# DavidPeicho/loupiote

Measured on AMD Instinct MI355X. Metric: Mrays/s (+ ms/frame) at 1920×1080, 4 spp, Sponza; 1/2/4/8 GPU, higher is better.
Workload: dtype f32

## Files before the change

loupiote_amd/csrc/device.hip:

```cpp
#include <hip/hip_runtime.h>

#include <dlfcn.h>

#include <algorithm>
#include <cmath>
#include <map>
#include <memory>
#include <cstdlib>
#include <functional>
#include <mutex>
#include <new>
#include <numeric>

#include "common.h"
#include "env_dist.h"
#include "emit_dist.h"
#include "material_tables.h"
#include "kernels.h"
#include "probe_kernels.h"
#include "build_kernels.h"
#include "launch_plan.h"
#include <hipcub/hipcub.hpp>
#include <rccl/rccl.h>

// ... 1887 lines not shown
                with_flags([&](auto D, auto L) { hipLaunchKernelGGL((k_raygen<decltype(D)::value, decltype(L)::value>), dim3(pl.stream_blocks), dim3(kBlock), 0, s, p, nz, w->q[0], w->Lsum, w->ctr); }, f.dense, f.lens);
                stage_end(r, s, slot);
                if (ph.wait_trav) HIP_TRY(hipStreamWaitEvent(s, ph.wait_trav, 0));
                if (pl.packet) {
                    stage_begin(r, ST_PRIMARY, s, slot);
                    with_flags([&](auto S) { hipLaunchKernelGGL(k_trace_packet<decltype(S)::value>, dim3(pl.packet_blocks), dim3(kTraceBlock), pl.packet_lds, s, sc, w->q[0], w->hits, w->ctr, 0, pl.quad_slots); }, f.stats);
                    stage_end(r, s, slot);
                } else if (pl.coop_all || !pl.path) trace(0, -1);
                if (pl.path) {
                    stage_begin(r, ST_PATH, s, slot);
                    const size_t plds = pl.stack_lds + kPathLdsExtra;
                    const float4 *h0 = pl.packet ? w->hits : (const float4 *)nullptr;
                    with_flags([&](auto G, auto S, auto P) {
                        auto launch = [&](auto... e) { hipLaunchKernelGGL((k_path<decltype(G)::value, decltype(S)::value, sizeof...(e) != 0, decltype(P)::value, decltype(e)...>), dim3(pl.path_blocks), dim3(kTraceBlock), plds, s, sc, probe, nz, p, w->q[0], h0, w->Lsum, w->ctr, seed0, gb, tune.path_refill, e...); };
                        if (f.env) launch(ev); else launch();
                    }, f.denoise, f.stats, f.punct);
                    stage_end(r, s, slot);
                }
            } else if (!pl.path) {
                const uint32_t b = t - 1u;
                const uint32_t seed = seed0 + t;
                const Queue qin = w->q[b & 1u], qout = w->q[(b + 1u) & 1u];
                stage_begin(r, ST_SHADE, s, slot);
                with_flags([&](auto G, auto P, auto Tr, auto Em, auto Es, auto Nm) {
                    auto launch = [&](auto... e) { hipLaunchKernelGGL((k_shade<decltype(G)::value, sizeof...(e) != 0, decltype(P)::value, decltype(Tr)::value, decltype(Em)::value, decltype(Em)::value && decltype(Es)::value, decltype(Nm)::value, decltype(e)...>), dim3(pl.shade_blocks), dim3(kBlock), 0, s, sc, probe, nz, p, qin, w->hits, qout, w->sq, w->Lsum, w->ctr, (int)b, seed, gb, sort_queues, e...); };
                    if (f.env) launch(ev); else launch();
                }, f.denoise && b == 0u, f.punct, f.trans, f.emis, esamp, f.nmap);
                stage_end(r, s, slot);
                if (ph.wait_trav) HIP_TRY(hipStreamWaitEvent(s, ph.wait_trav, 0));
                trace(b + 1u < nb ? (int)(b + 1u) : -1, (int)b);
            }
            if (ph.rec_trav) HIP_TRY(hipEventRecord(ph.rec_trav, s));
            if (t == nb && split) HIP_TRY(hipEventRecord(w->done, s));
            HIP_TRY(hipGetLastError());
            return LPT_OK;
        };
        for (uint32_t t = 0; !defer && t < tk.stages; ++t) {
            const int st = tk.run(t, PhaseHooks{});
            if (st != LPT_OK) return st;
        }
    }
    tk.p = p; tk.lane = lane; tk.split = split; tk.denoise = denoise; tk.cur = gb.cur;
    return LPT_OK;
}

static int wavefront_finish(lpt_renderer *r, const Ticket &tk, const ReadPlan *read, uint32_t row0, uint32_t row1) {
    hipStream_t sm = r->stream;
    const FrameParams &p = tk.p;
    Wavefront &wf = r->wf[tk.lane];
    const bool split = tk.split;
// ... 806 lines not shown
```

loupiote_amd/csrc/kernels.h:

```cpp
#pragma once
#include "device_math.h"

namespace lptd {

constexpr int kMaxBounces = 64;
constexpr int kBlock = 256;
constexpr int kTraceBlock = 64;

struct DNode8 {
    uint4 n0;
    uint4 n2;
    uint4 n3;
    uint4 n4;
};
using lpt::kNodeTris;

__device__ __forceinline__ uint32_t node_imask(const uint4 &n0) { return (n0.z >> 8) & 0xFFu; }
__device__ __forceinline__ uint32_t node_leaves(const uint4 &n0) { return n0.z >> 16; }
__device__ __forceinline__ uint32_t leaf_count(uint32_t V, uint32_t slot) { return 1u + ((V >> (8u + slot)) & 1u); }
struct NodeGrid { float px, py, pz, sx, sy, sz; };
template <typename Scene>
__device__ __forceinline__ NodeGrid node_grid(const Scene &sc, const uint4 &n0) {
    NodeGrid g;
    g.px = fmaf((float)(n0.x & 0xFFFFu), sc.grid_step[0], sc.grid_lo[0]);
// ... 143 lines not shown
        const uint32_t j = k - period * p.map.w;
#pragma unroll
        for (uint32_t q = 1; q < kMaxWeight; ++q) v = j == q ? p.map.vlist[q] : v;
    }
    const uint32_t tile = period * p.map.V + v;
    if (tile >= p.n_tiles) return false;
    const uint32_t ty = tile / p.tiles_x, tx = tile - ty * p.tiles_x;
    uint32_t wx, wy;
    within_to_xy(p, within, wx, wy);
    x = tx * p.tile_w + wx;
    y = ty * p.tile_h + wy;
    return x < p.width && y < p.height;
}

__device__ __forceinline__ uint32_t wave_compact(bool valid, uint32_t *counter) {
    const unsigned long long mask = __ballot(valid);
    const uint32_t lane = threadIdx.x & 63u;
    uint32_t base = 0;
    if (lane == 0 && mask) base = atomicAdd(counter, (uint32_t)__popcll(mask));
    base = __shfl(base, 0);
    return base + (uint32_t)__popcll(mask & ((1ull << lane) - 1ull));
}

__device__ __forceinline__ uint32_t block_compact(bool valid, uint32_t *counter, uint32_t *lds) {
    const unsigned long long mask = __ballot(valid);
    const uint32_t lane = threadIdx.x & 63u, wave = threadIdx.x >> 6;
    const uint32_t n = (uint32_t)__popcll(mask);
    if (lane == 0) lds[wave] = n;
    __syncthreads();
    if (threadIdx.x == 0) {
        const uint32_t n0 = lds[0], n1 = lds[1], n2 = lds[2], n3 = lds[3];
        const uint32_t total = n0 + n1 + n2 + n3;
        const uint32_t base = total ? atomicAdd(counter, total) : 0u;
        lds[4] = base; lds[5] = base + n0; lds[6] = base + n0 + n1; lds[7] = base + n0 + n1 + n2;
    }
    __syncthreads();
    const uint32_t idx = lds[4 + wave] + (uint32_t)__popcll(mask & ((1ull << lane) - 1ull));
    __syncthreads();
    return idx;
}

__device__ __forceinline__ uint32_t block_compact_binned(bool valid, uint32_t key, uint32_t *counter, uint32_t *lds) {
    const uint32_t lane = threadIdx.x & 63u, wave = threadIdx.x >> 6;
    unsigned long long mine = 0ull;
    uint32_t cnt_k = 0;
#pragma unroll
    for (uint32_t k = 0; k < 8u; ++k) {
        const unsigned long long m = __ballot(valid && key == k);
        if (key == k) mine = m;
        if (lane == k) cnt_k = (uint32_t)__popcll(m);
    }
    if (lane < 8u) lds[lane * 4u + wave] = cnt_k;
    __syncthreads();
    if (threadIdx.x < 32u) {
        const uint32_t c = lds[threadIdx.x];
        uint32_t incl = c;
#pragma unroll
        for (int off = 1; off < 32; off <<= 1) {
            const uint32_t v = __shfl_up(incl, off);
            if ((int)lane >= off) incl += v;
        }
        lds[32u + threadIdx.x] = incl - c;
        if (threadIdx.x == 31u) lds[64u] = incl ? atomicAdd(counter, incl) : 0u;
    }
    __syncthreads();
    const uint32_t idx = lds[64u] + lds[32u + key * 4u + wave] + (uint32_t)__popcll(mine & ((1ull << lane) - 1ull));
    __syncthreads();
    return idx;
}
__device__ __forceinline__ uint32_t dir_octant(float x, float y, float z) { return (x < 0.0f ? 1u : 0u) | (y < 0.0f ? 2u : 0u) | (z < 0.0f ? 4u : 0u); }

__device__ __forceinline__ void noise_shift(const DNoise &nz, uint32_t x, uint32_t y, uint32_t seed_counter, float &r0, float &r1) {
    if (!nz.enabled) return;
    const uint8_t *t = nz.rgba + 4u * ((size_t)(y % nz.h) * nz.w + (x % nz.w));
    float g = (float)(seed_counter & 1023u) * 0.61803398875f;
    float a = r0 + ((float)t[0] + 0.5f) * 0.00390625f + g;
    float b = r1 + ((float)t[1] + 0.5f) * 0.00390625f + g;
    a = a - floorf(a);
    b = b - floorf(b);
    if (a >= 1.0f) a = 0.0f;
    if (b >= 1.0f) b = 0.0f;
    r0 = a;
    r1 = b;
}

template <bool DENSE, bool LENS = false>
// ... 1197 lines not shown
    float4 no4, nd4, nT4;
    float4 so4, sd4, sc4;
};

struct PunctPick { float p_p, p_pick; };
template <bool ENV, bool ESAMP = false>
__device__ __forceinline__ PunctPick punct_pick(const DScene &sc) {
    PunctPick pk;
    pk.p_p = (float)sc.n_punctual / (float)(sc.n_punctual + sc.n_lights);
    pk.p_pick = (((ENV ? 0.5f : 1.0f) * (ESAMP ? 0.5f : 1.0f)) * pk.p_p) / (float)sc.n_punctual;
    return pk;
}
template <bool ENV, bool PUNCT, bool ESAMP = false>
__device__ __forceinline__ float rect_inv_nl(const DScene &sc, const PunctPick &pk) {
    if (PUNCT) return sc.n_lights ? (((ENV ? 0.5f : 1.0f) * (ESAMP ? 0.5f : 1.0f)) * (1.0f - pk.p_p)) / (float)sc.n_lights : 0.0f;
    return sc.n_lights ? ((ENV ? 0.5f : 1.0f) * (ESAMP ? 0.5f : 1.0f)) / (float)sc.n_lights : 0.0f;
}
template <bool ENV, bool ESAMP>
__device__ __forceinline__ float light_rl(const float r0, const float p_env, const float p_m) {
    float rl = ENV ? (r0 - p_env) / (1.0f - p_env) : r0;
    if (ESAMP) rl = (rl - p_m) / (1.0f - p_m);
    return rl;
}
template <bool GBUF, bool ENV, bool PUNCT, bool TRANS = false, bool EMIS = false, bool ESAMP = false, bool NMAP = false, typename LoadO, typename AddL>
__device__ __forceinline__ void shade_hit(const DScene &sc, const DProbe &probe, const DEnv &ev, const DNoise &nz, const FrameParams &p, const float *s_lut,
                                          const uint32_t bounce, const bool last_bounce, const uint32_t seed_base, const float inv_nl, const PunctPick &pk, const GBufArgs &gb,
                                          const float4 d4, const float4 T4, const float4 h4, LoadO load_o, AddL add_l, ShadeOut &out) {
    out.want_next = false; out.want_shadow = false; out.is_surface = false;
    const uint32_t pxy = __float_as_uint(T4.w);
    const f3 d = mk3(d4.x, d4.y, d4.z);
    const f3 T = mk3(T4.x, T4.y, T4.z);
    const uint32_t prim = __float_as_uint(h4.w);
    f3 g_n = neg(d), g_alb = mk3(1.0f, 1.0f, 1.0f);
    f3 g_P = mk3(0.f, 0.f, 0.f);
    if (GBUF && bounce == 0) {
        const float4 o4 = load_o();
        g_P = mk3(fmaf(d.x, h4.x, o4.x), fmaf(d.y, h4.x, o4.y), fmaf(d.z, h4.x, o4.z));
    }
    if (prim == 0xFFFFFFFFu) {
        f3 e = env_lookup(probe, d);
        if (ENV) {
            const float pdf_prev = load_o().w;
            if (pdf_prev >= 0.0f) {
                const float pe = ((PUNCT || ESAMP || sc.n_lights) ? 0.5f : 1.0f) * env_pdf(ev, d);
                const float pb2 = pdf_prev * pdf_prev;
                const float w = pb2 / (pb2 + pe * pe);
                e = mk3(e.x * w, e.y * w, e.z * w);
            }
        }
        add_l(T.x * e.x, T.y * e.y, T.z * e.z);
    } else if (prim & LPT_LIGHT_BIT) {
        const float4 *Lt = reinterpret_cast<const float4 *>(sc.lights + (prim & ~LPT_LIGHT_BIT));
        const float4 n4 = Lt[0], t4 = Lt[1], b4 = Lt[2], lo4 = Lt[3];
        const float Le = lo4.w;
        g_n = mk3(n4.x, n4.y, n4.z);
        float w = 1.0f;
        const float pdf_prev = load_o().w;
        if (pdf_prev >= 0.0f) {
            float cl = -dot(mk3(n4.x, n4.y, n4.z), d);
            float area = 4.0f * (t4.w * b4.w);
            float pl = ((h4.x * h4.x) / (cl * area)) * inv_nl;
            float pb2 = pdf_prev * pdf_prev;
            w = pb2 / (pb2 + pl * pl);
        }
        float k = Le * w;
        add_l(T.x * k, T.y * k, T.z * k);
    } else {
        const float hu = h4.y, hv = h4.z;
        const float4 *tv = sc.tri_verts + kTriRec * (size_t)prim;
        const float4 P0 = tv[0], N0 = tv[1], P1 = tv[2], N1 = tv[3], P2 = tv[4], N2 = tv[5];
        const float4 mc = tv[6], mp = tv[7];
        uint32_t em = 0u;
        if (EMIS) em = sc.emis_tri[prim];
        uint32_t nm = 0u;
        if (NMAP) nm = sc.nmap_tri[prim];
        float bw = (1.0f - hu) - hv;
        const f3 p0 = mk3(P0.x, P0.y, P0.z), p1 = mk3(P1.x, P1.y, P1.z), p2 = mk3(P2.x, P2.y, P2.z);
        f3 P = mk3((p0.x * bw + p1.x * hu) + p2.x * hv, (p0.y * bw + p1.y * hu) + p2.y * hv, (p0.z * bw + p1.z * hu) + p2.z * hv);
        f3 Ng = cross(p1 - p0, p2 - p0);
        float l2 = dot(Ng, Ng);
        if (l2 > 0.0f) {
            out.is_surface = true;
            Ng = Ng * (1.0f / sqrtf(l2));
            f3 Ns = mk3((N0.x * bw + N1.x * hu) + N2.x * hv, (N0.y * bw + N1.y * hu) + N2.y * hv, (N0.z * bw + N1.z * hu) + N2.z * hv);
            float n2 = dot(Ns, Ns);
            Ns = n2 > 0.0f ? Ns * (1.0f / sqrtf(n2)) : Ng;
            const bool entering = !(dot(Ng, d) > 0.0f);
            if (dot(Ng, d) > 0.0f) Ng = neg(Ng);
            const f3 Nv = Ns;
            const bool flip = dot(Ns, Ng) < 0.0f;
            if (flip) Ns = neg(Ns);
            float tu = (P0.w * bw + P1.w * hu) + P2.w * hv;
            float tvv = (N0.w * bw + N1.w * hu) + N2.w * hv;
            if (NMAP && nm != 0u) normal_map(sc, s_lut, nm, Nv, Ng, flip, p1 - p0, p2 - p0, P1.w - P0.w, N1.w - N0.w, P2.w - P0.w, N2.w - N0.w, tu, tvv, Ns);
            f3 base = mk3(mc.x, mc.y, mc.z);
            float rough = mp.x, metal = mp.y;
            const uint32_t atex = __float_as_uint(mp.z), mtex = __float_as_uint(mp.w);
            if ((atex >> 30) == 1u) {
                f3 alb;
                float mg, mb;
                texture_lookup_pair(sc, s_lut, atex & ~kPairedBit, mtex, tu, tvv, alb, mg, mb);
                base.x *= alb.x; base.y *= alb.y; base.z *= alb.z;
                rough *= mg; metal *= mb;
            } else {
                if (atex < sc.n_images) {
                    const float4 tex = texture_lookup(sc, s_lut, atex, tu, tvv, true);
                    base.x *= tex.x; base.y *= tex.y; base.z *= tex.z;
                }
                if (mtex < sc.n_images) {
                    const float4 tex = texture_lookup(sc, s_lut, mtex, tu, tvv, false);
                    rough *= tex.y; metal *= tex.z;
                }
            }
            if (EMIS && em != 0u) {
                const float4 er = sc.emis_recs[em - 1u];
                f3 E = mk3(er.x, er.y, er.z);
                const uint32_t etex = __float_as_uint(er.w);
                if (etex < sc.n_images) {
                    const float4 tex = texture_lookup(sc, s_lut, etex, tu, tvv, true);
                    E.x *= tex.x; E.y *= tex.y; E.z *= tex.z;
                }
                if (ESAMP) {
                    const float pdf_prev = load_o().w;
                    if (pdf_prev >= 0.0f) {
                        const float cl = fabsf(dot(Ng, d));
                        const float pA = lum(mk3(er.x, er.y, er.z)) * sc.emit_inv_W;
                        const float p_sel = (ENV ? 0.5f : 1.0f) * ((PUNCT || sc.n_lights) ? 0.5f : 1.0f);
                        const float pl = (((h4.x * h4.x) / cl) * pA) * p_sel;
                        const float pb2 = pdf_prev * pdf_prev;
                        const float w = pb2 / (pb2 + pl * pl);
                        E = mk3(E.x * w, E.y * w, E.z * w);
                    }
                }
                add_l(T.x * E.x, T.y * E.y, T.z * E.z);
            }
            g_n = Ns; g_P = P;
            g_alb = mk3(clampf(base.x, 0.0f, 1.0f), clampf(base.y, 0.0f, 1.0f), clampf(base.z, 0.0f, 1.0f));
            const Surface sf = make_surface(base, rough, metal);
            const f3 V = neg(d);
            const float NoV = max2(dot(Ns, V), LPT_MIN_NOV);
            const float pspec = spec_probability(sf, NoV);
            const uint32_t x = pxy & 0x1FFFu, y = (pxy >> 13) & 0x1FFFu, sample = pxy >> 26;
            const uint32_t pixel = y * p.width + x;
            const uint32_t seed_counter = seed_base + sample * p.max_bounces;
            Rng rg = rng_init(pixel, stage_seed(p.user_seed, seed_counter), LPT_TAG_SHADE);
            float r0 = rng_next(rg), r1 = rng_next(rg), r2 = rng_next(rg);
            float r3 = rng_next(rg), r4 = rng_next(rg), r5 = rng_next(rg);
            noise_shift(nz, x, y, seed_counter, r4, r5);
            float r6 = 0.0f, r7 = 0.0f, r8 = 0.0f, r9 = 0.0f;
            if (ENV) { r6 = rng_next(rg); r7 = rng_next(rg); r8 = rng_next(rg); r9 = rng_next(rg); }
            float ra = 0.0f, rb = 0.0f;
            if (ESAMP) { ra = rng_next(rg); rb = rng_next(rg); }
            const float p_env = (PUNCT || ESAMP || sc.n_lights) ? 0.5f : 1.0f;
            const float p_m = (PUNCT || sc.n_lights) ? 0.5f : 1.0f;
            float am = max2(max2(fabsf(P.x), fabsf(P.y)), fabsf(P.z));
            float eps = 1.0e-4f * (1.0f + am);
            const f3 Po = mk3(P.x + Ng.x * eps, P.y + Ng.y * eps, P.z + Ng.z * eps);
            bool glass = false;
            if (TRANS) {
                const uint32_t te = sc.trans_tri[prim];
                if (te != 0u) {
                    const float4 tr = sc.trans_recs[te - 1u];
                    const float pt = tr.x * (1.0f - clampf(metal, 0.0f, 1.0f));
                    if (r3 < pt) {
                        glass = true;
                        if (!last_bounce) {
                            const InterfaceOut io = interface_sample(d, Ns, Ng, entering, base, tr.y, tr.z != 0.0f, r4);
                            const f3 Tn = mk3(T.x * io.weight.x, T.y * io.weight.y, T.z * io.weight.z);
                            if (Tn.x > 0.0f || Tn.y > 0.0f || Tn.z > 0.0f) {
                                const f3 Pn = io.transmit ? mk3(P.x - Ng.x * eps, P.y - Ng.y * eps, P.z - Ng.z * eps) : Po;
                                out.want_next = true;
                                out.no4 = make_float4(Pn.x, Pn.y, Pn.z, -1.0f);
                                out.nd4 = make_float4(io.wi.x, io.wi.y, io.wi.z, d4.w);
                                out.nT4 = make_float4(Tn.x, Tn.y, Tn.z, T4.w);
                            }
                        }
                    } else {
                        r3 = (r3 - pt) / (1.0f - pt);
                    }
                }
            }
            if (TRANS && glass) {
            } else if (ENV && r0 < p_env) {
                f3 wi;
                float ps;
                if (env_sample(ev, r6, r7, r8, r9, r1, r2, wi, ps)) {
                    Hit hl;
                    hl.t = LPT_T_INF; hl.u = 0.f; hl.v = 0.f; hl.prim = 0xFFFFFFFFu;
                    intersect_lights(sc, Po, wi, hl);
                    if (hl.prim == 0xFFFFFFFFu) {
                        f3 f;
                        float pb;
                        bsdf_eval(sf, Ns, Ng, V, NoV, pspec, wi, f, pb);
                        if (pb > 0.0f) {
                            const f3 Le = env_lookup(probe, wi);
                            const float pe = p_env * env_pdf(ev, wi);
                            const float pe2 = pe * pe;
                            const float wm = last_bounce ? 1.0f : pe2 / (pe2 + pb * pb);
                            const float NoL = dot(Ns, wi);
                            const float k = (NoL * wm) / (p_env * ps);
                            f3 contrib = mk3(((T.x * f.x) * Le.x) * k, ((T.y * f.y) * Le.y) * k, ((T.z * f.z) * Le.z) * k);
                            if (contrib.x > 0.0f || contrib.y > 0.0f || contrib.z > 0.0f) {
                                out.want_shadow = true;
                                out.so4 = make_float4(Po.x, Po.y, Po.z, LPT_T_INF);
                                out.sd4 = make_float4(wi.x, wi.y, wi.z, d4.w);
                                out.sc4 = make_float4(contrib.x, contrib.y, contrib.z, 0.f);
                            }
                        }
                    }
                }
            } else if (ESAMP && light_rl<ENV, false>(r0, p_env, p_m) < p_m) {
                EmitterSample es;
                if (!last_bounce && emitter_sample(sc, s_lut, ra, rb, r1, r2, Po, es)) {
                    Hit hl;
                    hl.t = es.dist; hl.u = 0.f; hl.v = 0.f; hl.prim = 0xFFFFFFFFu;
                    intersect_lights(sc, Po, es.wi, hl);
                    if (hl.prim == 0xFFFFFFFFu) {
                        f3 f;
                        float pb;
                        bsdf_eval(sf, Ns, Ng, V, NoV, pspec, es.wi, f, pb);
                        if (pb > 0.0f) {
                            const float pl = ((es.d2 / es.cl) * es.pA) * ((ENV ? 0.5f : 1.0f) * p_m);
                            const float pl2 = pl * pl;
                            const float wm = pl2 / (pl2 + pb * pb);
                            const float NoL = dot(Ns, es.wi);
                            f3 contrib = mk3((T.x * f.x) * (((NoL * es.E.x) * wm) / pl), (T.y * f.y) * (((NoL * es.E.y) * wm) / pl), (T.z * f.z) * (((NoL * es.E.z) * wm) / pl));
                            if (contrib.x > 0.0f || contrib.y > 0.0f || contrib.z > 0.0f) {
                                out.want_shadow = true;
                                out.so4 = make_float4(Po.x, Po.y, Po.z, es.dist * 0.999f);
                                out.sd4 = make_float4(es.wi.x, es.wi.y, es.wi.z, d4.w);
                                out.sc4 = make_float4(contrib.x, contrib.y, contrib.z, 0.f);
                            }
                        }
                    }
                }
            } else if (PUNCT && light_rl<ENV, ESAMP>(r0, p_env, p_m) < pk.p_p) {
                const float rl = light_rl<ENV, ESAMP>(r0, p_env, p_m);
                uint32_t li = (uint32_t)((rl / pk.p_p) * (float)sc.n_punctual);
                if (li > sc.n_punctual - 1u) li = sc.n_punctual - 1u;
                f3 wi, E;
                float dist;
                if (punctual_sample(sc, li, Po, wi, dist, E)) {
                    Hit hl;
                    hl.t = dist; hl.u = 0.f; hl.v = 0.f; hl.prim = 0xFFFFFFFFu;
                    intersect_lights(sc, Po, wi, hl);
                    if (hl.prim == 0xFFFFFFFFu) {
                        f3 f;
                        float pb;
                        bsdf_eval(sf, Ns, Ng, V, NoV, pspec, wi, f, pb);
                        if (pb > 0.0f) {
                            const float NoL = dot(Ns, wi);
                            f3 contrib = mk3((T.x * f.x) * ((NoL * E.x) / pk.p_pick), (T.y * f.y) * ((NoL * E.y) / pk.p_pick), (T.z * f.z) * ((NoL * E.z) / pk.p_pick));
                            if (contrib.x > 0.0f || contrib.y > 0.0f || contrib.z > 0.0f) {
                                out.want_shadow = true;
                                out.so4 = make_float4(Po.x, Po.y, Po.z, dist < LPT_T_INF ? dist * 0.999f : LPT_T_INF);
                                out.sd4 = make_float4(wi.x, wi.y, wi.z, d4.w);
                                out.sc4 = make_float4(contrib.x, contrib.y, contrib.z, 0.f);
                            }
                        }
                    }
                }
            } else if (sc.n_lights) {
                float rl = light_rl<ENV, ESAMP>(r0, p_env, p_m);
                if (PUNCT) rl = (rl - pk.p_p) / (1.0f - pk.p_p);
                uint32_t li = (uint32_t)(rl * (float)sc.n_lights);
                if (li > sc.n_lights - 1u) li = sc.n_lights - 1u;
                const float4 *Lt = reinterpret_cast<const float4 *>(sc.lights + li);
                const float4 n4 = Lt[0], t4 = Lt[1], b4 = Lt[2], lo4 = Lt[3];
                const float Le = lo4.w, hw = t4.w, hh = b4.w;
                float a = (2.0f * r1 - 1.0f) * hw, bq = (2.0f * r2 - 1.0f) * hh;
                f3 qp = mk3((lo4.x + t4.x * a) + b4.x * bq, (lo4.y + t4.y * a) + b4.y * bq, (lo4.z + t4.z * a) + b4.z * bq);
                f3 w = qp - Po;
                float d2 = dot(w, w);
                if (Le > 0.0f && d2 > 0.0f) {
                    float dist = sqrtf(d2);
                    f3 wi = w * (1.0f / dist);
                    float cl = -dot(mk3(n4.x, n4.y, n4.z), wi);
                    if (cl > 0.0f) {
                        f3 f;
                        float pb;
                        bsdf_eval(sf, Ns, Ng, V, NoV, pspec, wi, f, pb);
                        if (pb > 0.0f) {
                            float area = 4.0f * (hw * hh);
                            float pl = (d2 / (cl * area)) * inv_nl;
                            float pl2 = pl * pl;
                            float wm = pl2 / (pl2 + pb * pb);
                            float NoL = dot(Ns, wi);
                            float k = ((NoL * Le) * wm) / pl;
                            f3 contrib = mk3((T.x * f.x) * k, (T.y * f.y) * k, (T.z * f.z) * k);
                            if (contrib.x > 0.0f || contrib.y > 0.0f || contrib.z > 0.0f) {
// ... 2 lines not shown
                                out.sd4 = make_float4(wi.x, wi.y, wi.z, d4.w);
                                out.sc4 = make_float4(contrib.x, contrib.y, contrib.z, 0.f);
                            }
                        }
                    }
                }
            }
            if (!last_bounce && !(TRANS && glass)) {
                f3 Ln, wgt;
                float pdf;
                if (bsdf_sample(sf, Ns, Ng, V, NoV, pspec, r3, r4, r5, Ln, wgt, pdf)) {
                    f3 Tn = mk3(T.x * wgt.x, T.y * wgt.y, T.z * wgt.z);
                    if (Tn.x > 0.0f || Tn.y > 0.0f || Tn.z > 0.0f) {
                        out.want_next = true;
                        out.no4 = make_float4(Po.x, Po.y, Po.z, pdf);
                        out.nd4 = make_float4(Ln.x, Ln.y, Ln.z, d4.w);
                        out.nT4 = make_float4(Tn.x, Tn.y, Tn.z, T4.w);
                    }
                }
            }
        }
    }
    if (GBUF && bounce == 0) {
        const uint32_t gx = pxy & 0x1FFFu, gy = (pxy >> 13) & 0x1FFFu;
        const size_t px = (size_t)gy * p.width + gx;
        gb.gbuf[px] = make_uint4(prim, __float_as_uint(h4.x), oct_encode(g_n), pack_albedo(g_alb));
        float mu = 0.0f, mv = 0.0f, cu, cv, pu, pv;
        if (prim != 0xFFFFFFFFu && project(gb.cur, g_P, cu, cv) && project(gb.prev, g_P, pu, pv)) { mu = pu - cu; mv = pv - cv; }
        gb.motion[px] = make_float2(mu, mv);
    }
}

#ifndef LPT_SHADE_WAVES
#define LPT_SHADE_WAVES(ENV, PUNCT) (((ENV) || (PUNCT)) ? 3 : 4)
#endif
#ifndef LPT_SHADE_WAVES_TRANS
#define LPT_SHADE_WAVES_TRANS(ENV, PUNCT) 3
#endif
#ifndef LPT_SHADE_WAVES_EMIS
#define LPT_SHADE_WAVES_EMIS(ENV, PUNCT, TRANS) 3
#endif
#ifndef LPT_SHADE_WAVES_ESAMP
#define LPT_SHADE_WAVES_ESAMP(ENV, PUNCT, TRANS) 3
#endif
#ifndef LPT_SHADE_WAVES_NMAP
#define LPT_SHADE_WAVES_NMAP(ENV, PUNCT, TRANS, EMIS, ESAMP) 3
#endif
template <bool GBUF, bool ENV = false, bool PUNCT = false, bool TRANS = false, bool EMIS = false, bool ESAMP = false, bool NMAP = false, typename... Env>
__global__ __launch_bounds__(kBlock) __attribute__((amdgpu_waves_per_eu(NMAP ? LPT_SHADE_WAVES_NMAP(ENV, PUNCT, TRANS, EMIS, ESAMP) : ESAMP ? LPT_SHADE_WAVES_ESAMP(ENV, PUNCT, TRANS) : EMIS ? LPT_SHADE_WAVES_EMIS(ENV, PUNCT, TRANS) : TRANS ? LPT_SHADE_WAVES_TRANS(ENV, PUNCT) : LPT_SHADE_WAVES(ENV, PUNCT)))) void k_shade(DScene sc, DProbe probe, DNoise nz, FrameParams p, Queue qin, const float4 *hits,
                                                  Queue qout, ShadowQueue sq, float4 *Lsum, FrameCounters *ctr, int bounce,
                                                  uint32_t seed_base, GBufArgs gb, int sorted, Env... env) {
    static_assert(sizeof...(Env) == (ENV ? 1u : 0u), "the ENV instantiations take the distribution, the others nothing");
    static_assert(EMIS || !ESAMP, "emitter sampling (SPEC §23) exists only for a scene with an emissive material in use");
    const DEnv ev = env_arg(env...);
    __shared__ uint32_t lds[72];
    __shared__ float s_lut[256];
    __shared__ float4 s_park[6 * kBlock];
    __shared__ uint32_t s_at[2 * kBlock];
    s_lut[threadIdx.x] = sc.srgb_lut[threadIdx.x];
    __syncthreads();
    bool parked = false;
    const uint32_t count = QC(ctr, bounce);
    const uint32_t stride = gridDim.x * blockDim.x;
    const uint32_t rounded = (count + 255u) & ~255u;
    uint32_t n_surface = 0;
    const bool last_bounce = (uint32_t)bounce + 1u >= p.max_bounces;
    const PunctPick pk = PUNCT ? punct_pick<ENV, ESAMP>(sc) : PunctPick{0.0f, 0.0f};
    const float inv_nl = rect_inv_nl<ENV, PUNCT, ESAMP>(sc, pk);
    for (uint32_t i0 = blockIdx.x * blockDim.x + threadIdx.x; i0 < rounded; i0 += stride) {
        ShadeOut so;
        so.want_next = false; so.want_shadow = false; so.is_surface = false;
        const uint32_t i = i0;
        if (i < count) {
            const float4 d4 = ld_nt(qin.d + i), T4 = ld_nt(qin.T + i), h4 = ld_nt(hits + i);
            const uint32_t slot = __float_as_uint(d4.w);
            shade_hit<GBUF, ENV, PUNCT, TRANS, EMIS, ESAMP, NMAP>(sc, probe, ev, nz, p, s_lut, (uint32_t)bounce, last_bounce, seed_base, inv_nl, pk, gb, d4, T4, h4,
                            [&]() { return ld_nt(qin.o + i); },
                            [&](float r, float g, float b) {
                                float4 L = Lsum[slot];
                                L.x = L.x + r; L.y = L.y + g; L.z = L.z + b;
                                Lsum[slot] = L;
                            }, so);
        }
        if (!(sorted & 3)) {
            const bool va = so.want_shadow, vb = so.want_next && !last_bounce;
            const unsigned long long ma = __ballot(va), mb = __ballot(vb);
            const uint32_t lane = threadIdx.x & 63u, wave = threadIdx.x >> 6;
            const unsigned long long lt = (1ull << lane) - 1ull;
            const uint32_t wa = (uint32_t)__popcll(ma & lt), wb = (uint32_t)__popcll(mb & lt);
            if (!parked && i0 + stride < rounded) {
                if (lane == 0) lds[16 + wave] = (uint32_t)__popcll(ma) | ((uint32_t)__popcll(mb) << 16);
                s_at[threadIdx.x] = va ? wa : 0xFFFFFFFFu;
                s_at[kBlock + threadIdx.x] = vb ? wb : 0xFFFFFFFFu;
                if (va) { s_park[threadIdx.x] = so.so4; s_park[kBlock + threadIdx.x] = so.sd4; s_park[2 * kBlock + threadIdx.x] = so.sc4; }
                if (vb) { s_park[3 * kBlock + threadIdx.x] = so.no4; s_park[4 * kBlock + threadIdx.x] = so.nd4; s_park[5 * kBlock + threadIdx.x] = so.nT4; }
                parked = true;
            } else {
                if (lane == 0) lds[wave] = (uint32_t)__popcll(ma) | ((uint32_t)__popcll(mb) << 16);
                __syncthreads();
                if (threadIdx.x == 0) {
                    uint32_t ra = 0u, rb = 0u;
                    for (uint32_t w = 0; w < 8u; ++w) {
                        const uint32_t c = w < 4u ? (parked ? lds[16 + w] : 0u) : lds[w - 4u];
                        lds[24 + w] = ra; lds[32 + w] = rb;
                        ra += c & 0xFFFFu; rb += c >> 16;
                    }
                    unsigned long long base = 0ull;
                    if (ra | rb) base = atomicAdd(reinterpret_cast<unsigned long long *>(&SC(ctr, bounce)), (unsigned long long)ra | ((unsigned long long)rb << 32));
                    lds[40] = (uint32_t)base; lds[41] = (uint32_t)(base >> 32);
                }
                __syncthreads();
                if (parked) {
                    const uint32_t pa = s_at[threadIdx.x], pb = s_at[kBlock + threadIdx.x];
                    if (pa != 0xFFFFFFFFu) {
                        const uint32_t si = lds[40] + lds[24 + wave] + pa;
                        st_nt(sq.o + si, s_park[threadIdx.x]); st_nt(sq.d + si, s_park[kBlock + threadIdx.x]); st_nt(sq.c + si, s_park[2 * kBlock + threadIdx.x]);
                    }
                    if (pb != 0xFFFFFFFFu) {
                        const uint32_t ni = lds[41] + lds[32 + wave] + pb;
                        st_nt(qout.o + ni, s_park[3 * kBlock + threadIdx.x]); st_nt(qout.d + ni, s_park[4 * kBlock + threadIdx.x]); st_nt(qout.T + ni, s_park[5 * kBlock + threadIdx.x]);
                    }
                }
                if (va) { const uint32_t si = lds[40] + lds[28 + wave] + wa; st_nt(sq.o + si, so.so4); st_nt(sq.d + si, so.sd4); st_nt(sq.c + si, so.sc4); }
                if (vb) { const uint32_t ni = lds[41] + lds[36 + wave] + wb; st_nt(qout.o + ni, so.no4); st_nt(qout.d + ni, so.nd4); st_nt(qout.T + ni, so.nT4); }
                __syncthreads();
                parked = false;
            }
        } else {
            const uint32_t si = (sorted & 2) ? block_compact_binned(so.want_shadow, so.want_shadow ? dir_octant(so.sd4.x, so.sd4.y, so.sd4.z) : 0u, &SC(ctr, bounce), lds)
                                       : block_compact(so.want_shadow, &SC(ctr, bounce), lds);
            if (so.want_shadow) { st_nt(sq.o + si, so.so4); st_nt(sq.d + si, so.sd4); st_nt(sq.c + si, so.sc4); }
            if (!last_bounce) {
                const uint32_t ni = (sorted & 1) ? block_compact_binned(so.want_next, so.want_next ? dir_octant(so.nd4.x, so.nd4.y, so.nd4.z) : 0u, &QC(ctr, bounce + 1), lds)
                                           : block_compact(so.want_next, &QC(ctr, bounce + 1), lds);
                if (so.want_next) { st_nt(qout.o + ni, so.no4); st_nt(qout.d + ni, so.nd4); st_nt(qout.T + ni, so.nT4); }
            }
        }
        n_surface += so.is_surface ? 1u : 0u;
    }
    for (int off = 32; off > 0; off >>= 1) n_surface += __shfl_down(n_surface, off);
    if ((threadIdx.x & 63u) == 0) lds[threadIdx.x >> 6] = n_surface;
    __syncthreads();
    if (threadIdx.x == 0) {
        const uint32_t total = (lds[0] + lds[1]) + (lds[2] + lds[3]);
        if (total) atomicAdd(&ctr->shaded_part[((uint32_t)bounce * 8u + (blockIdx.x & 7u)) * 32u], total);
    }
}

#ifndef LPT_PATH_WAVES
#define LPT_PATH_WAVES(ENV, PUNCT) (((ENV) || (PUNCT)) ? 3 : 4)
#endif
constexpr uint32_t kPathLdsExtra = 1024u + 3u * kMaxBounces * 4u;
template <bool GBUF, bool STATS, bool ENV = false, bool PUNCT = false, typename... Env>
__global__ __launch_bounds__(kTraceBlock) __attribute__((amdgpu_waves_per_eu(LPT_PATH_WAVES(ENV, PUNCT), LPT_PATH_WAVES(ENV, PUNCT)))) void k_path(
        DScene sc, DProbe probe, DNoise nz, FrameParams p, Queue q0, const float4 *hits0, float4 *Lsum, FrameCounters *ctr, uint32_t seed0, GBufArgs gb, int refill,
        Env... env) {
    static_assert(sizeof...(Env) == (ENV ? 1u : 0u), "the ENV instantiations take the distribution, the others nothing");
    const DEnv ev = env_arg(env...);
    static_assert(kTraceBlock == 64, "one wave per block: the LDS hand-overs below are ordered by the wave's own program order");
    uint2 *stack = reinterpret_cast<uint2 *>(lds_dyn) + threadIdx.x;
    const uint32_t stack_bytes = sc.stack_entries * kTraceBlock * (uint32_t)sizeof(uint2);
    float *s_lut = reinterpret_cast<float *>(lds_dyn + stack_bytes);
    uint32_t *s_cnt = reinterpret_cast<uint32_t *>(lds_dyn + stack_bytes + 1024u);
    const uint32_t lane = threadIdx.x;
#pragma unroll
    for (int k = 0; k < 4; ++k) s_lut[lane + 64u * k] = sc.srgb_lut[lane + 64u * k];
#pragma unroll
    for (int k = 0; k < 3; ++k) s_cnt[lane + 64u * k] = 0u;
// ... 31 lines not shown
                    const float4 d4 = ld_nt(q0.d + idx);
                    pxy = __float_as_uint(q0.T[idx].w);
                    vslot = __float_as_uint(d4.w);
                    T = mk3(1.f, 1.f, 1.f); L = mk3(0.f, 0.f, 0.f);
                    pdf = -1.0f; bounce = 0u;
                    if (hits0) {
                        const float4 h4 = ld_nt(hits0 + idx);
                        rs.o = p.origin; rs.d = mk3(d4.x, d4.y, d4.z);
                        rs.best.t = h4.x; rs.best.u = h4.y; rs.best.v = h4.z; rs.best.prim = __float_as_uint(h4.w);
                        phase = 2u;
                    } else {
                        ray_begin(sc, rs, p.origin, mk3(d4.x, d4.y, d4.z), LPT_T_INF);
                        shadow = false;
                        phase = 1u;
                    }
                }
                pl.next = min(pl.end, pl.next + (uint32_t)__popcll(imask));
            }
            if (phase == 2u) {
                ShadeOut so;
                const float4 d4 = make_float4(rs.d.x, rs.d.y, rs.d.z, __uint_as_float(vslot));
                const float4 T4 = make_float4(T.x, T.y, T.z, __uint_as_float(pxy));
                const float4 h4 = make_float4(rs.best.t, rs.best.u, rs.best.v, __uint_as_float(rs.best.prim));
                shade_hit<GBUF, ENV, PUNCT>(sc, probe, ev, nz, p, s_lut, bounce, bounce + 1u >= nb, seed0 + bounce + 1u, inv_nl, pk, gb, d4, T4, h4,
                                [&]() { return make_float4(rs.o.x, rs.o.y, rs.o.z, pdf); },
                                [&](float r, float g, float b) { L.x = L.x + r; L.y = L.y + g; L.z = L.z + b; }, so);
                if (so.is_surface) atomicAdd(&s_cnt[128u + bounce], 1u);
                if (so.want_shadow) atomicAdd(&s_cnt[64u + bounce], 1u);
                if (so.want_next) {
                    atomicAdd(&s_cnt[bounce + 1u], 1u);
                    T = mk3(so.nT4.x, so.nT4.y, so.nT4.z);
                    pdf = so.no4.w;
                    nd = mk3(so.nd4.x, so.nd4.y, so.nd4.z);
                }
                has_next = so.want_next;
                if (so.want_shadow) {
                    ray_begin(sc, rs, mk3(so.so4.x, so.so4.y, so.so4.z), mk3(so.sd4.x, so.sd4.y, so.sd4.z), so.so4.w);
                    cs = mk3(so.sc4.x, so.sc4.y, so.sc4.z);
                    shadow = true;
                    phase = 1u;
                } else if (so.want_next) {
                    ray_begin(sc, rs, mk3(so.no4.x, so.no4.y, so.no4.z), nd, LPT_T_INF);
                    shadow = false;
                    bounce++;
                    phase = 1u;
                } else {
                    Lsum[vslot] = make_float4(L.x, L.y, L.z, 0.0f);
                    phase = 0u;
                }
// ... 458 lines not shown
```

Measured before the change: 6335.

## Reload cold shade kernel arguments from kernarg segment to cut SGPR pressure

k_shade now takes a single struct argument. Rarely used fields (probe, noise, gbuf, lights, output queues, counters) are re-read through an opaque kernarg segment pointer at their point of use instead of being held live across the shading body. The aim is to shrink scalar and vector register live ranges in the shade kernel, which could reduce spills or allow higher occupancy. The cost is extra scalar loads from the kernarg segment, and the asm volatile barriers may restrict some optimisation.

```diff
diff --git a/loupiote_amd/csrc/device.hip b/loupiote_amd/csrc/device.hip
--- a/loupiote_amd/csrc/device.hip
+++ b/loupiote_amd/csrc/device.hip
@@ -1933,10 +1933,10 @@
                 const uint32_t seed = seed0 + t;
                 const Queue qin = w->q[b & 1u], qout = w->q[(b + 1u) & 1u];
                 stage_begin(r, ST_SHADE, s, slot);
-                with_flags([&](auto G, auto P, auto Tr, auto Em, auto Es, auto Nm) {
-                    auto launch = [&](auto... e) { hipLaunchKernelGGL((k_shade<decltype(G)::value, sizeof...(e) != 0, decltype(P)::value, decltype(Tr)::value, decltype(Em)::value, decltype(Em)::value && decltype(Es)::value, decltype(Nm)::value, decltype(e)...>), dim3(pl.shade_blocks), dim3(kBlock), 0, s, sc, probe, nz, p, qin, w->hits, qout, w->sq, w->Lsum, w->ctr, (int)b, seed, gb, sort_queues, e...); };
-                    if (f.env) launch(ev); else launch();
-                }, f.denoise && b == 0u, f.punct, f.trans, f.emis, esamp, f.nmap);
+                const ShadeKernargs ska{sc, probe, nz, p, qin, w->hits, qout, w->sq, w->Lsum, w->ctr, (int)b, seed, gb, sort_queues, ev};
+                with_flags([&](auto G, auto E, auto P, auto Tr, auto Em, auto Es, auto Nm) {
+                    hipLaunchKernelGGL((k_shade<decltype(G)::value, decltype(E)::value, decltype(P)::value, decltype(Tr)::value, decltype(Em)::value, decltype(Em)::value && decltype(Es)::value, decltype(Nm)::value>), dim3(pl.shade_blocks), dim3(kBlock), 0, s, ska);
+                }, f.denoise && b == 0u, f.env, f.punct, f.trans, f.emis, esamp, f.nmap);
                 stage_end(r, s, slot);
                 if (ph.wait_trav) HIP_TRY(hipStreamWaitEvent(s, ph.wait_trav, 0));
                 trace(b + 1u < nb ? (int)(b + 1u) : -1, (int)b);
diff --git a/loupiote_amd/csrc/kernels.h b/loupiote_amd/csrc/kernels.h
--- a/loupiote_amd/csrc/kernels.h
+++ b/loupiote_amd/csrc/kernels.h
@@ -189,13 +189,13 @@
     return base + (uint32_t)__popcll(mask & ((1ull << lane) - 1ull));
 }
 
-__device__ __forceinline__ uint32_t block_compact(bool valid, uint32_t *counter, uint32_t *lds) {
+__device__ __forceinline__ uint32_t block_compact(bool valid, uint32_t *counter, uint32_t *lds, const uint32_t tid = threadIdx.x) {
     const unsigned long long mask = __ballot(valid);
-    const uint32_t lane = threadIdx.x & 63u, wave = threadIdx.x >> 6;
+    const uint32_t lane = tid & 63u, wave = tid >> 6;
     const uint32_t n = (uint32_t)__popcll(mask);
     if (lane == 0) lds[wave] = n;
     __syncthreads();
-    if (threadIdx.x == 0) {
+    if (tid == 0) {
         const uint32_t n0 = lds[0], n1 = lds[1], n2 = lds[2], n3 = lds[3];
         const uint32_t total = n0 + n1 + n2 + n3;
         const uint32_t base = total ? atomicAdd(counter, total) : 0u;
@@ -207,8 +207,8 @@
     return idx;
 }
 
-__device__ __forceinline__ uint32_t block_compact_binned(bool valid, uint32_t key, uint32_t *counter, uint32_t *lds) {
-    const uint32_t lane = threadIdx.x & 63u, wave = threadIdx.x >> 6;
+__device__ __forceinline__ uint32_t block_compact_binned(bool valid, uint32_t key, uint32_t *counter, uint32_t *lds, const uint32_t tid = threadIdx.x) {
+    const uint32_t lane = tid & 63u, wave = tid >> 6;
     unsigned long long mine = 0ull;
     uint32_t cnt_k = 0;
 #pragma unroll
@@ -219,16 +219,16 @@
     }
     if (lane < 8u) lds[lane * 4u + wave] = cnt_k;
     __syncthreads();
-    if (threadIdx.x < 32u) {
-        const uint32_t c = lds[threadIdx.x];
+    if (tid < 32u) {
+        const uint32_t c = lds[tid];
         uint32_t incl = c;
 #pragma unroll
         for (int off = 1; off < 32; off <<= 1) {
             const uint32_t v = __shfl_up(incl, off);
             if ((int)lane >= off) incl += v;
         }
-        lds[32u + threadIdx.x] = incl - c;
-        if (threadIdx.x == 31u) lds[64u] = incl ? atomicAdd(counter, incl) : 0u;
+        lds[32u + tid] = incl - c;
+        if (tid == 31u) lds[64u] = incl ? atomicAdd(counter, incl) : 0u;
     }
     __syncthreads();
     const uint32_t idx = lds[64u] + lds[32u + key * 4u + wave] + (uint32_t)__popcll(mine & ((1ull << lane) - 1ull));
@@ -1472,10 +1472,11 @@
     if (ESAMP) rl = (rl - p_m) / (1.0f - p_m);
     return rl;
 }
-template <bool GBUF, bool ENV, bool PUNCT, bool TRANS = false, bool EMIS = false, bool ESAMP = false, bool NMAP = false, typename LoadO, typename AddL>
-__device__ __forceinline__ void shade_hit(const DScene &sc, const DProbe &probe, const DEnv &ev, const DNoise &nz, const FrameParams &p, const float *s_lut,
-                                          const uint32_t bounce, const bool last_bounce, const uint32_t seed_base, const float inv_nl, const PunctPick &pk, const GBufArgs &gb,
-                                          const float4 d4, const float4 T4, const float4 h4, LoadO load_o, AddL add_l, ShadeOut &out) {
+struct ShadeCold { const DScene &sc; const DProbe &probe; const DNoise &nz; const GBufArgs &gb; };
+template <bool GBUF, bool ENV, bool PUNCT, bool TRANS = false, bool EMIS = false, bool ESAMP = false, bool NMAP = false, typename LoadO, typename AddL, typename Cold>
+__device__ __forceinline__ void shade_hit(const DScene &sc, const DEnv &ev, const FrameParams &p, const float *s_lut,
+                                          const uint32_t bounce, const bool last_bounce, const uint32_t seed_base, const float inv_nl, const PunctPick &pk,
+                                          const float4 d4, const float4 T4, const float4 h4, LoadO load_o, AddL add_l, Cold cold, ShadeOut &out) {
     out.want_next = false; out.want_shadow = false; out.is_surface = false;
     const uint32_t pxy = __float_as_uint(T4.w);
     const f3 d = mk3(d4.x, d4.y, d4.z);
@@ -1488,11 +1489,12 @@
         g_P = mk3(fmaf(d.x, h4.x, o4.x), fmaf(d.y, h4.x, o4.y), fmaf(d.z, h4.x, o4.z));
     }
     if (prim == 0xFFFFFFFFu) {
-        f3 e = env_lookup(probe, d);
+        const ShadeCold c = cold();
+        f3 e = env_lookup(c.probe, d);
         if (ENV) {
             const float pdf_prev = load_o().w;
             if (pdf_prev >= 0.0f) {
-                const float pe = ((PUNCT || ESAMP || sc.n_lights) ? 0.5f : 1.0f) * env_pdf(ev, d);
+                const float pe = ((PUNCT || ESAMP || c.sc.n_lights) ? 0.5f : 1.0f) * env_pdf(ev, d);
                 const float pb2 = pdf_prev * pdf_prev;
                 const float w = pb2 / (pb2 + pe * pe);
                 e = mk3(e.x * w, e.y * w, e.z * w);
@@ -1500,7 +1502,7 @@
         }
         add_l(T.x * e.x, T.y * e.y, T.z * e.z);
     } else if (prim & LPT_LIGHT_BIT) {
-        const float4 *Lt = reinterpret_cast<const float4 *>(sc.lights + (prim & ~LPT_LIGHT_BIT));
+        const float4 *Lt = reinterpret_cast<const float4 *>(cold().sc.lights + (prim & ~LPT_LIGHT_BIT));
         const float4 n4 = Lt[0], t4 = Lt[1], b4 = Lt[2], lo4 = Lt[3];
         const float Le = lo4.w;
         g_n = mk3(n4.x, n4.y, n4.z);
@@ -1542,28 +1544,30 @@
             if (flip) Ns = neg(Ns);
             float tu = (P0.w * bw + P1.w * hu) + P2.w * hv;
             float tvv = (N0.w * bw + N1.w * hu) + N2.w * hv;
-            if (NMAP && nm != 0u) normal_map(sc, s_lut, nm, Nv, Ng, flip, p1 - p0, p2 - p0, P1.w - P0.w, N1.w - N0.w, P2.w - P0.w, N2.w - N0.w, tu, tvv, Ns);
+            if (NMAP && nm != 0u) normal_map(cold().sc, s_lut, nm, Nv, Ng, flip, p1 - p0, p2 - p0, P1.w - P0.w, N1.w - N0.w, P2.w - P0.w, N2.w - N0.w, tu, tvv, Ns);
             f3 base = mk3(mc.x, mc.y, mc.z);
             float rough = mp.x, metal = mp.y;
             const uint32_t atex = __float_as_uint(mp.z), mtex = __float_as_uint(mp.w);
+            const DScene &ts = cold().sc;
             if ((atex >> 30) == 1u) {
                 f3 alb;
                 float mg, mb;
-                texture_lookup_pair(sc, s_lut, atex & ~kPairedBit, mtex, tu, tvv, alb, mg, mb);
+                texture_lookup_pair(ts, s_lut, atex & ~kPairedBit, mtex, tu, tvv, alb, mg, mb);
                 base.x *= alb.x; base.y *= alb.y; base.z *= alb.z;
                 rough *= mg; metal *= mb;
             } else {
-                if (atex < sc.n_images) {
-                    const float4 tex = texture_lookup(sc, s_lut, atex, tu, tvv, true);
+                if (atex < ts.n_images) {
+                    const float4 tex = texture_lookup(ts, s_lut, atex, tu, tvv, true);
                     base.x *= tex.x; base.y *= tex.y; base.z *= tex.z;
                 }
-                if (mtex < sc.n_images) {
-                    const float4 tex = texture_lookup(sc, s_lut, mtex, tu, tvv, false);
+                if (mtex < ts.n_images) {
+                    const float4 tex = texture_lookup(ts, s_lut, mtex, tu, tvv, false);
                     rough *= tex.y; metal *= tex.z;
                 }
             }
             if (EMIS && em != 0u) {
-                const float4 er = sc.emis_recs[em - 1u];
+                const DScene &cs = cold().sc;
+                const float4 er = cs.emis_recs[em - 1u];
                 f3 E = mk3(er.x, er.y, er.z);
                 const uint32_t etex = __float_as_uint(er.w);
                 if (etex < sc.n_images) {
@@ -1574,8 +1578,8 @@
                     const float pdf_prev = load_o().w;
                     if (pdf_prev >= 0.0f) {
                         const float cl = fabsf(dot(Ng, d));
-                        const float pA = lum(mk3(er.x, er.y, er.z)) * sc.emit_inv_W;
-                        const float p_sel = (ENV ? 0.5f : 1.0f) * ((PUNCT || sc.n_lights) ? 0.5f : 1.0f);
+                        const float pA = lum(mk3(er.x, er.y, er.z)) * cs.emit_inv_W;
+                        const float p_sel = (ENV ? 0.5f : 1.0f) * ((PUNCT || cs.n_lights) ? 0.5f : 1.0f);
                         const float pl = (((h4.x * h4.x) / cl) * pA) * p_sel;
                         const float pb2 = pdf_prev * pdf_prev;
                         const float w = pb2 / (pb2 + pl * pl);
@@ -1596,21 +1600,23 @@
             Rng rg = rng_init(pixel, stage_seed(p.user_seed, seed_counter), LPT_TAG_SHADE);
             float r0 = rng_next(rg), r1 = rng_next(rg), r2 = rng_next(rg);
             float r3 = rng_next(rg), r4 = rng_next(rg), r5 = rng_next(rg);
-            noise_shift(nz, x, y, seed_counter, r4, r5);
+            const ShadeCold c = cold();
+            const DScene &cs = c.sc;
+            noise_shift(c.nz, x, y, seed_counter, r4, r5);
             float r6 = 0.0f, r7 = 0.0f, r8 = 0.0f, r9 = 0.0f;
             if (ENV) { r6 = rng_next(rg); r7 = rng_next(rg); r8 = rng_next(rg); r9 = rng_next(rg); }
             float ra = 0.0f, rb = 0.0f;
             if (ESAMP) { ra = rng_next(rg); rb = rng_next(rg); }
-            const float p_env = (PUNCT || ESAMP || sc.n_lights) ? 0.5f : 1.0f;
-            const float p_m = (PUNCT || sc.n_lights) ? 0.5f : 1.0f;
+            const float p_env = (PUNCT || ESAMP || cs.n_lights) ? 0.5f : 1.0f;
+            const float p_m = (PUNCT || cs.n_lights) ? 0.5f : 1.0f;
             float am = max2(max2(fabsf(P.x), fabsf(P.y)), fabsf(P.z));
             float eps = 1.0e-4f * (1.0f + am);
             const f3 Po = mk3(P.x + Ng.x * eps, P.y + Ng.y * eps, P.z + Ng.z * eps);
             bool glass = false;
             if (TRANS) {
-                const uint32_t te = sc.trans_tri[prim];
+                const uint32_t te = cs.trans_tri[prim];
                 if (te != 0u) {
-                    const float4 tr = sc.trans_recs[te - 1u];
+                    const float4 tr = cs.trans_recs[te - 1u];
                     const float pt = tr.x * (1.0f - clampf(metal, 0.0f, 1.0f));
                     if (r3 < pt) {
                         glass = true;
@@ -1637,13 +1643,13 @@
                 if (env_sample(ev, r6, r7, r8, r9, r1, r2, wi, ps)) {
                     Hit hl;
                     hl.t = LPT_T_INF; hl.u = 0.f; hl.v = 0.f; hl.prim = 0xFFFFFFFFu;
-                    intersect_lights(sc, Po, wi, hl);
+                    intersect_lights(cs, Po, wi, hl);
                     if (hl.prim == 0xFFFFFFFFu) {
                         f3 f;
                         float pb;
                         bsdf_eval(sf, Ns, Ng, V, NoV, pspec, wi, f, pb);
                         if (pb > 0.0f) {
-                            const f3 Le = env_lookup(probe, wi);
+                            const f3 Le = env_lookup(c.probe, wi);
                             const float pe = p_env * env_pdf(ev, wi);
                             const float pe2 = pe * pe;
                             const float wm = last_bounce ? 1.0f : pe2 / (pe2 + pb * pb);
@@ -1661,10 +1667,10 @@
                 }
             } else if (ESAMP && light_rl<ENV, false>(r0, p_env, p_m) < p_m) {
                 EmitterSample es;
-                if (!last_bounce && emitter_sample(sc, s_lut, ra, rb, r1, r2, Po, es)) {
+                if (!last_bounce && emitter_sample(cs, s_lut, ra, rb, r1, r2, Po, es)) {
                     Hit hl;
                     hl.t = es.dist; hl.u = 0.f; hl.v = 0.f; hl.prim = 0xFFFFFFFFu;
-                    intersect_lights(sc, Po, es.wi, hl);
+                    intersect_lights(cs, Po, es.wi, hl);
                     if (hl.prim == 0xFFFFFFFFu) {
                         f3 f;
                         float pb;
@@ -1686,14 +1692,14 @@
                 }
             } else if (PUNCT && light_rl<ENV, ESAMP>(r0, p_env, p_m) < pk.p_p) {
                 const float rl = light_rl<ENV, ESAMP>(r0, p_env, p_m);
-                uint32_t li = (uint32_t)((rl / pk.p_p) * (float)sc.n_punctual);
-                if (li > sc.n_punctual - 1u) li = sc.n_punctual - 1u;
+                uint32_t li = (uint32_t)((rl / pk.p_p) * (float)cs.n_punctual);
+                if (li > cs.n_punctual - 1u) li = cs.n_punctual - 1u;
                 f3 wi, E;
                 float dist;
-                if (punctual_sample(sc, li, Po, wi, dist, E)) {
+                if (punctual_sample(cs, li, Po, wi, dist, E)) {
                     Hit hl;
                     hl.t = dist; hl.u = 0.f; hl.v = 0.f; hl.prim = 0xFFFFFFFFu;
-                    intersect_lights(sc, Po, wi, hl);
+                    intersect_lights(cs, Po, wi, hl);
                     if (hl.prim == 0xFFFFFFFFu) {
                         f3 f;
                         float pb;
@@ -1710,12 +1716,12 @@
                         }
                     }
                 }
-            } else if (sc.n_lights) {
+            } else if (cs.n_lights) {
                 float rl = light_rl<ENV, ESAMP>(r0, p_env, p_m);
                 if (PUNCT) rl = (rl - pk.p_p) / (1.0f - pk.p_p);
-                uint32_t li = (uint32_t)(rl * (float)sc.n_lights);
-                if (li > sc.n_lights - 1u) li = sc.n_lights - 1u;
-                const float4 *Lt = reinterpret_cast<const float4 *>(sc.lights + li);
+                uint32_t li = (uint32_t)(rl * (float)cs.n_lights);
+                if (li > cs.n_lights - 1u) li = cs.n_lights - 1u;
+                const float4 *Lt = reinterpret_cast<const float4 *>(cs.lights + li);
                 const float4 n4 = Lt[0], t4 = Lt[1], b4 = Lt[2], lo4 = Lt[3];
                 const float Le = lo4.w, hw = t4.w, hh = b4.w;
                 float a = (2.0f * r1 - 1.0f) * hw, bq = (2.0f * r2 - 1.0f) * hh;
@@ -1764,6 +1770,7 @@
         }
     }
     if (GBUF && bounce == 0) {
+        const GBufArgs &gb = cold().gb;
         const uint32_t gx = pxy & 0x1FFFu, gy = (pxy >> 13) & 0x1FFFu;
         const size_t px = (size_t)gy * p.width + gx;
         gb.gbuf[px] = make_uint4(prim, __float_as_uint(h4.x), oct_encode(g_n), pack_albedo(g_alb));
@@ -1773,6 +1780,16 @@
     }
 }
 
+struct ShadeKernargs {
+    DScene sc; DProbe probe; DNoise nz; FrameParams p; Queue qin; const float4 *hits; Queue qout; ShadowQueue sq; float4 *Lsum; FrameCounters *ctr;
+    int bounce; uint32_t seed_base; GBufArgs gb; int sorted; DEnv ev;
+};
+typedef const __attribute__((address_space(4))) ShadeKernargs *ShadeKernargsPtr;
+__device__ __forceinline__ ShadeKernargsPtr shade_kernargs() {
+    ShadeKernargsPtr ka = (ShadeKernargsPtr)__builtin_amdgcn_kernarg_segment_ptr();
+    asm volatile("" : "+s"(ka));
+    return ka;
+}
 #ifndef LPT_SHADE_WAVES
 #define LPT_SHADE_WAVES(ENV, PUNCT) (((ENV) || (PUNCT)) ? 3 : 4)
 #endif
@@ -1788,13 +1805,14 @@
 #ifndef LPT_SHADE_WAVES_NMAP
 #define LPT_SHADE_WAVES_NMAP(ENV, PUNCT, TRANS, EMIS, ESAMP) 3
 #endif
-template <bool GBUF, bool ENV = false, bool PUNCT = false, bool TRANS = false, bool EMIS = false, bool ESAMP = false, bool NMAP = false, typename... Env>
-__global__ __launch_bounds__(kBlock) __attribute__((amdgpu_waves_per_eu(NMAP ? LPT_SHADE_WAVES_NMAP(ENV, PUNCT, TRANS, EMIS, ESAMP) : ESAMP ? LPT_SHADE_WAVES_ESAMP(ENV, PUNCT, TRANS) : EMIS ? LPT_SHADE_WAVES_EMIS(ENV, PUNCT, TRANS) : TRANS ? LPT_SHADE_WAVES_TRANS(ENV, PUNCT) : LPT_SHADE_WAVES(ENV, PUNCT)))) void k_shade(DScene sc, DProbe probe, DNoise nz, FrameParams p, Queue qin, const float4 *hits,
-                                                  Queue qout, ShadowQueue sq, float4 *Lsum, FrameCounters *ctr, int bounce,
-                                                  uint32_t seed_base, GBufArgs gb, int sorted, Env... env) {
-    static_assert(sizeof...(Env) == (ENV ? 1u : 0u), "the ENV instantiations take the distribution, the others nothing");
+template <bool GBUF, bool ENV = false, bool PUNCT = false, bool TRANS = false, bool EMIS = false, bool ESAMP = false, bool NMAP = false>
+__global__ __launch_bounds__(kBlock) __attribute__((amdgpu_waves_per_eu(NMAP ? LPT_SHADE_WAVES_NMAP(ENV, PUNCT, TRANS, EMIS, ESAMP) : ESAMP ? LPT_SHADE_WAVES_ESAMP(ENV, PUNCT, TRANS) : EMIS ? LPT_SHADE_WAVES_EMIS(ENV, PUNCT, TRANS) : TRANS ? LPT_SHADE_WAVES_TRANS(ENV, PUNCT) : LPT_SHADE_WAVES(ENV, PUNCT)))) void k_shade(const ShadeKernargs a) {
     static_assert(EMIS || !ESAMP, "emitter sampling (SPEC §23) exists only for a scene with an emissive material in use");
-    const DEnv ev = env_arg(env...);
+    const DScene &sc = a.sc;
+    const FrameParams &p = a.p;
+    const float4 *const qin_d = a.qin.d, *const qin_T = a.qin.T, *const hits = a.hits;
+    const int bounce = a.bounce, sorted = a.sorted;
+    const uint32_t seed_base = a.seed_base;
     __shared__ uint32_t lds[72];
     __shared__ float s_lut[256];
     __shared__ float4 s_park[6 * kBlock];
@@ -1802,7 +1820,7 @@
     s_lut[threadIdx.x] = sc.srgb_lut[threadIdx.x];
     __syncthreads();
     bool parked = false;
-    const uint32_t count = QC(ctr, bounce);
+    const uint32_t count = QC(a.ctr, bounce);
     const uint32_t stride = gridDim.x * blockDim.x;
     const uint32_t rounded = (count + 255u) & ~255u;
     uint32_t n_surface = 0;
@@ -1814,15 +1832,17 @@
         so.want_next = false; so.want_shadow = false; so.is_surface = false;
         const uint32_t i = i0;
         if (i < count) {
-            const float4 d4 = ld_nt(qin.d + i), T4 = ld_nt(qin.T + i), h4 = ld_nt(hits + i);
+            const float4 d4 = ld_nt(qin_d + i), T4 = ld_nt(qin_T + i), h4 = ld_nt(hits + i);
             const uint32_t slot = __float_as_uint(d4.w);
-            shade_hit<GBUF, ENV, PUNCT, TRANS, EMIS, ESAMP, NMAP>(sc, probe, ev, nz, p, s_lut, (uint32_t)bounce, last_bounce, seed_base, inv_nl, pk, gb, d4, T4, h4,
-                            [&]() { return ld_nt(qin.o + i); },
+            shade_hit<GBUF, ENV, PUNCT, TRANS, EMIS, ESAMP, NMAP>(sc, a.ev, p, s_lut, (uint32_t)bounce, last_bounce, seed_base, inv_nl, pk, d4, T4, h4,
+                            [&]() { return ld_nt(shade_kernargs()->qin.o + i); },
                             [&](float r, float g, float b) {
+                                float4 *const Lsum = shade_kernargs()->Lsum;
                                 float4 L = Lsum[slot];
                                 L.x = L.x + r; L.y = L.y + g; L.z = L.z + b;
                                 Lsum[slot] = L;
-                            }, so);
+                            },
+                            []() { const ShadeKernargs *k = (const ShadeKernargs *)shade_kernargs(); return ShadeCold{k->sc, k->probe, k->nz, k->gb}; }, so);
         }
         if (!(sorted & 3)) {
             const bool va = so.want_shadow, vb = so.want_next && !last_bounce;
@@ -1838,6 +1858,11 @@
                 if (vb) { s_park[3 * kBlock + threadIdx.x] = so.no4; s_park[4 * kBlock + threadIdx.x] = so.nd4; s_park[5 * kBlock + threadIdx.x] = so.nT4; }
                 parked = true;
             } else {
+                ShadeKernargsPtr ka = shade_kernargs();
+                FrameCounters *const ctr = ka->ctr;
+                const int bounce = ka->bounce;
+                Queue qout; qout.o = ka->qout.o; qout.d = ka->qout.d; qout.T = ka->qout.T;
+                ShadowQueue sq; sq.o = ka->sq.o; sq.d = ka->sq.d; sq.c = ka->sq.c;
                 if (lane == 0) lds[wave] = (uint32_t)__popcll(ma) | ((uint32_t)__popcll(mb) << 16);
                 __syncthreads();
                 if (threadIdx.x == 0) {
@@ -1869,12 +1894,19 @@
                 parked = false;
             }
         } else {
-            const uint32_t si = (sorted & 2) ? block_compact_binned(so.want_shadow, so.want_shadow ? dir_octant(so.sd4.x, so.sd4.y, so.sd4.z) : 0u, &SC(ctr, bounce), lds)
-                                       : block_compact(so.want_shadow, &SC(ctr, bounce), lds);
+            ShadeKernargsPtr ka = shade_kernargs();
+            FrameCounters *const ctr = ka->ctr;
+            Queue qout; qout.o = ka->qout.o; qout.d = ka->qout.d; qout.T = ka->qout.T;
+            ShadowQueue sq; sq.o = ka->sq.o; sq.d = ka->sq.d; sq.c = ka->sq.c;
+            const int bounce = ka->bounce, sorted = ka->sorted;
+            uint32_t tid = threadIdx.x;
+            asm volatile("" : "+v"(tid));
+            const uint32_t si = (sorted & 2) ? block_compact_binned(so.want_shadow, so.want_shadow ? dir_octant(so.sd4.x, so.sd4.y, so.sd4.z) : 0u, &SC(ctr, bounce), lds, tid)
+                                       : block_compact(so.want_shadow, &SC(ctr, bounce), lds, tid);
             if (so.want_shadow) { st_nt(sq.o + si, so.so4); st_nt(sq.d + si, so.sd4); st_nt(sq.c + si, so.sc4); }
             if (!last_bounce) {
-                const uint32_t ni = (sorted & 1) ? block_compact_binned(so.want_next, so.want_next ? dir_octant(so.nd4.x, so.nd4.y, so.nd4.z) : 0u, &QC(ctr, bounce + 1), lds)
-                                           : block_compact(so.want_next, &QC(ctr, bounce + 1), lds);
+                const uint32_t ni = (sorted & 1) ? block_compact_binned(so.want_next, so.want_next ? dir_octant(so.nd4.x, so.nd4.y, so.nd4.z) : 0u, &QC(ctr, bounce + 1), lds, tid)
+                                           : block_compact(so.want_next, &QC(ctr, bounce + 1), lds, tid);
                 if (so.want_next) { st_nt(qout.o + ni, so.no4); st_nt(qout.d + ni, so.nd4); st_nt(qout.T + ni, so.nT4); }
             }
         }
@@ -1885,7 +1917,7 @@
     __syncthreads();
     if (threadIdx.x == 0) {
         const uint32_t total = (lds[0] + lds[1]) + (lds[2] + lds[3]);
-        if (total) atomicAdd(&ctr->shaded_part[((uint32_t)bounce * 8u + (blockIdx.x & 7u)) * 32u], total);
+        if (total) atomicAdd(&shade_kernargs()->ctr->shaded_part[((uint32_t)bounce * 8u + (blockIdx.x & 7u)) * 32u], total);
     }
 }
 
@@ -1963,9 +1995,10 @@
                 const float4 d4 = make_float4(rs.d.x, rs.d.y, rs.d.z, __uint_as_float(vslot));
                 const float4 T4 = make_float4(T.x, T.y, T.z, __uint_as_float(pxy));
                 const float4 h4 = make_float4(rs.best.t, rs.best.u, rs.best.v, __uint_as_float(rs.best.prim));
-                shade_hit<GBUF, ENV, PUNCT>(sc, probe, ev, nz, p, s_lut, bounce, bounce + 1u >= nb, seed0 + bounce + 1u, inv_nl, pk, gb, d4, T4, h4,
+                shade_hit<GBUF, ENV, PUNCT>(sc, ev, p, s_lut, bounce, bounce + 1u >= nb, seed0 + bounce + 1u, inv_nl, pk, d4, T4, h4,
                                 [&]() { return make_float4(rs.o.x, rs.o.y, rs.o.z, pdf); },
-                                [&](float r, float g, float b) { L.x = L.x + r; L.y = L.y + g; L.z = L.z + b; }, so);
+                                [&](float r, float g, float b) { L.x = L.x + r; L.y = L.y + g; L.z = L.z + b; },
+                                [&]() { return ShadeCold{sc, probe, nz, gb}; }, so);
                 if (so.is_surface) atomicAdd(&s_cnt[128u + bounce], 1u);
                 if (so.want_shadow) atomicAdd(&s_cnt[64u + bounce], 1u);
                 if (so.want_next) {
```

After: 6412, median of 6. 1.01x the previous value.
